# emmyoh/zebra

Hardware: AMD Instinct MI355X
Metric: queries/sec (higher is better)
Workload: dtype f32

## Files before the change

zebra_amd/csrc/zh_approx.hip:

```cpp

#include <cstdlib>

#include "zh_internal.h"
#include "zh_device.h"

typedef _Float16 f16x8 __attribute__((ext_vector_type(8)));

#ifndef ZH_APX_G768
#define ZH_APX_G768 2
#endif
#ifndef ZH_APX_G128
#define ZH_APX_G128 8
#endif
uint32_t zh_approx_groups(uint32_t d) {
    switch (d) {
    case 128: return ZH_APX_G128;
    case 256: case 384: return 4;
    case 768: return ZH_APX_G768;
    case 512: case 1024: return 2;
    default: return 0;
    }
}
bool zh_approx_pays(uint32_t d) { return d >= 384; }

float zh_approx_bound(int metric, uint32_t d, int mfma) {
    const double u = 5.9604644775390625e-8, c0 = (d + 255) / 256 + 8.0, ops = mfma ? 33.0 * (d / 128) + 2.0 + (mfma == 2 ? 40.0 : 0.0) : 0.0;
    if (metric == ZH_COSINE) return (float)(1.01 * (2.0 * c0 + 80.0 + 2.0 * ops) * u);
    return (float)(1.01 * (c0 + 100.0 + ops) * u);
}

__device__ __forceinline__ _Float16 f16_no_subnormal(float v) {
    const _Float16 h = (_Float16)v;
    return fabsf((float)h) < 6.103515625e-05f ? (_Float16)0.f : h;
}

template <int G>
__global__ __launch_bounds__(64) void qhalf_kernel(const float *__restrict__ Q, uint32_t B, uint32_t d, _Float16 *__restrict__ Qh,
                                                    float4 *__restrict__ qmeta) {
    constexpr uint32_t LG = 64 / G;
    const uint32_t b = blockIdx.x, lane = threadIdx.x;
    const float *q = Q + (size_t)b * d;
    float m = 0.f, s2 = 0.f;
    bool bad = false;
    for (uint32_t e = lane; e < d; e += 64) {
        const float v = q[e];
        bad |= !(v - v == 0.f);
        m = fmaxf(m, fabsf(v));
        s2 = __builtin_fmaf(v, v, s2);
    }
    m = wave_butterfly<OpMax>(m);
    s2 = wave_sum_canonical(s2);
    bad = __ballot(bad) != 0;
    float sigma = 1.f, inv = 1.f;
    if (!bad && m > 0.f) {
        int ex = 0;
        (void)frexpf(m, &ex);
        if (ex < -90 || ex > 90) bad = true;
        else { sigma = ldexpf(1.f, 14 - ex); inv = ldexpf(1.f, ex - 14); }
    }
    float d2 = 0.f;
    for (uint32_t e = lane; e < d; e += 64) {
        const float v = bad ? 0.f : q[e];
        const _Float16 h = f16_no_subnormal(v * sigma);
        const float df = v - (float)h * inv;
        d2 = __builtin_fmaf(df, df, d2);
        const uint32_t j = e / (4 * LG), rem = e % (4 * LG), l = rem / 4, t = rem % 4, i = j / 2, wh = j % 2;
        Qh[(size_t)b * d + ((size_t)(i * LG + l)) * 8 + wh * 4 + t] = h;
    }
    d2 = wave_sum_canonical(d2);
    if (lane == 0) {
        float4 o;
        if (bad || !(s2 - s2 == 0.f)) o = make_float4(NAN, NAN, NAN, NAN);
        else o = make_float4(inv, s2, sqrtf(s2) * (1.0f + 1e-5f), sqrtf(d2) * 1.001f);
        qmeta[b] = o;
    }
}

hipError_t zh_launch_qhalf(const float *dQ, uint32_t B, uint32_t d, void *dQh, float4 *dQmeta, int layout, hipStream_t s) {
    if (!B) return hipSuccess;
    const uint32_t G = layout == 2 ? 64 : (layout == 1 ? 16 : zh_approx_groups(d));
    if (G == 64) hipLaunchKernelGGL(qhalf_kernel<64>, dim3(B), dim3(64), 0, s, dQ, B, d, (_Float16 *)dQh, dQmeta);
    else if (G == 16) hipLaunchKernelGGL(qhalf_kernel<16>, dim3(B), dim3(64), 0, s, dQ, B, d, (_Float16 *)dQh, dQmeta);
    else if (G == 8) hipLaunchKernelGGL(qhalf_kernel<8>, dim3(B), dim3(64), 0, s, dQ, B, d, (_Float16 *)dQh, dQmeta);
    else if (G == 4) hipLaunchKernelGGL(qhalf_kernel<4>, dim3(B), dim3(64), 0, s, dQ, B, d, (_Float16 *)dQh, dQmeta);
    else if (G == 2) hipLaunchKernelGGL(qhalf_kernel<2>, dim3(B), dim3(64), 0, s, dQ, B, d, (_Float16 *)dQh, dQmeta);
    else return hipErrorInvalidValue;
    return hipGetLastError();
}

template <int LG>
__device__ __forceinline__ float group_sum(float s) {
    s = s + dpp_mov<0xB1>(s);
    s = s + dpp_mov<0x4E>(s);
    s = s + dpp_mov<0x141>(s);
    if (LG >= 16) s = s + dpp_mov<0x140>(s);
    if (LG >= 32) s = xor16<OpAdd>(s);
    if (LG >= 64) {
        const auto r = __builtin_amdgcn_permlane32_swap(__float_as_uint(s), __float_as_uint(s), false, false);
        s = __uint_as_float(r[0]) + __uint_as_float(r[1]);
    }
    return s;
}


__device__ __forceinline__ uint32_t scan_phase1(uint32_t lane, uint32_t n_ent, const uint2 *__restrict__ ent,
                                                const uint32_t *__restrict__ visitBits, const uint4 *__restrict__ nodeVisit,
                                                uint32_t *eGb, uint32_t *eWithin, uint32_t *eC, uint32_t *off, uint32_t *eB0, uint64_t *eK0) {
    unsigned long long rlw[ZH_SCAN_NE];
#pragma unroll
    for (int j = 0; j < ZH_SCAN_NE; j++) {
        const uint32_t e = lane + 64u * j;
        rlw[j] = __builtin_nontemporal_load(reinterpret_cast<const unsigned long long *>(ent + (e < n_ent ? e : 0)));
    }
    uint32_t word[ZH_SCAN_NE];
    bool in[ZH_SCAN_NE];
#pragma unroll
    for (int j = 0; j < ZH_SCAN_NE; j++) {
        const uint32_t node = (uint32_t)rlw[j];
        in[j] = lane + 64u * j < n_ent && node != 0xFFFFFFFFu;
        word[j] = visitBits[in[j] ? node >> 5 : 0];
    }
    uint4 nv[ZH_SCAN_NE];
#pragma unroll
    for (int j = 0; j < ZH_SCAN_NE; j++) {
        const uint32_t node = (uint32_t)rlw[j];
        in[j] = in[j] && ((word[j] >> (node & 31)) & 1u);
        nv[j] = nodeVisit[in[j] ? node : 0];
    }
    uint32_t P = 0;
#pragma unroll
    for (int j = 0; j < ZH_SCAN_NE; j++) {
        eWithin[j] = (uint32_t)(rlw[j] >> 32);
        eC[j] = in[j] ? nv[j].x & 0x0FFFFFFFu : 0u;
        eGb[j] = nv[j].y; eB0[j] = nv[j].z;
        eK0[j] = ((uint64_t)(nv[j].x >> 28) << 32) | nv[j].w;
        uint32_t incl = eC[j];
#pragma unroll
        for (int o = 1; o < 64; o <<= 1) {
            const uint32_t t = __shfl_up(incl, o);
            if (lane >= (uint32_t)o) incl += t;
        }
        off[j] = P + incl - eC[j];
        P += (uint32_t)__builtin_amdgcn_readlane((int)incl, 63);
    }
    return P;
}

#define ZH_APX_CAP 512
#ifndef ZH_APX_WAVES
#define ZH_APX_WAVES 0
#endif
#ifndef ZH_APX_REPL_ROWS
#define ZH_APX_REPL_ROWS 0
#endif
template <int D, int G, int KINDA>
__global__ __launch_bounds__(256)
#if ZH_APX_WAVES
__attribute__((amdgpu_waves_per_eu(ZH_APX_WAVES, 8)))
#endif
void scan_approx_kernel(const float *__restrict__ X, const uint4 *__restrict__ Qh,
                                                           const float4 *__restrict__ qmeta, const uint2 *__restrict__ rowLeaf,
                                                           uint32_t T, uint32_t RW, const uint32_t *__restrict__ visitBits,
                                                           const uint4 *__restrict__ nodeVisit, const ZhGroup *__restrict__ groups,
                                                           uint32_t GRP, uint64_t row_begin, uint64_t row_end, float Kc,
                                                           uint64_t *__restrict__ iv) {
    constexpr int LG = 64 / G, NH = D * G / 512, NR = 2 * NH;
    constexpr int RB = NR <= 6 ? 4 : 2;
    static_assert(D * G % 512 == 0 && NH >= 1, "a lane's share of a query is whole 16-byte loads");
    __shared__ uint4 pair_list[4][ZH_APX_CAP];
    __shared__ uint32_t row_start[4][20];
    const uint32_t lane = threadIdx.x & 63, l = lane & (LG - 1), g = lane / LG;
    const uint32_t wid = (uint32_t)__builtin_amdgcn_readfirstlane((int)(threadIdx.x >> 6));
    const uint64_t wave = (uint64_t)blockIdx.x * (blockDim.x >> 6) + wid;
    const uint64_t r0 = row_begin + wave * RW;
    if (r0 >= row_end) return;
    const uint32_t nr = (uint32_t)(row_end - r0 < RW ? row_end - r0 : RW);
    const uint32_t n_ent = nr * T;
    const uint2 *__restrict__ ent = rowLeaf + (size_t)r0 * T;
    uint32_t eGb[ZH_SCAN_NE], eWithin[ZH_SCAN_NE], eC[ZH_SCAN_NE], off[ZH_SCAN_NE], eB0[ZH_SCAN_NE];
    uint64_t eK0[ZH_SCAN_NE];
    const uint32_t P = scan_phase1(lane, n_ent, ent, visitBits, nodeVisit, eGb, eWithin, eC, off, eB0, eK0);
    if (P == 0) return;
    const float4 *__restrict__ X4 = reinterpret_cast<const float4 *>(X);
    float my_s = 0.f, my_a2 = 0.f;
    uint64_t my_slot = 0;
    uint32_t nst = 0;
    bool my_on = false;
    auto flush = [&]() {
        if (my_on) __builtin_nontemporal_store(((uint64_t)__float_as_uint(my_a2) << 32) | __float_as_uint(my_s), iv + my_slot);
        my_on = false;
        nst = 0;
    };
    auto load_q = [&](uint32_t b, uint4 *hq) {
        const uint4 *qp = Qh + (size_t)b * (D / 8) + l;
#pragma unroll
        for (int i = 0; i < NH; i++) hq[i] = qp[i * LG];
    };
    auto load_x = [&](uint64_t row, float4 *v) {
        if constexpr (G == 2 && !ZH_APX_REPL_ROWS) {
            const float4 *r4 = X4 + (size_t)row * (D / 4) + lane;
#pragma unroll
            for (int j = 0; j < NR / 2; j++) {
                const float4 t = ld16<true>(r4 + 64 * j);
                const auto sx = __builtin_amdgcn_permlane32_swap(__float_as_uint(t.x), __float_as_uint(t.x), false, false);
                const auto sy = __builtin_amdgcn_permlane32_swap(__float_as_uint(t.y), __float_as_uint(t.y), false, false);
                const auto sz = __builtin_amdgcn_permlane32_swap(__float_as_uint(t.z), __float_as_uint(t.z), false, false);
                const auto sw = __builtin_amdgcn_permlane32_swap(__float_as_uint(t.w), __float_as_uint(t.w), false, false);
                v[2 * j] = make_float4(__uint_as_float(sx[0]), __uint_as_float(sy[0]), __uint_as_float(sz[0]), __uint_as_float(sw[0]));
                v[2 * j + 1] = make_float4(__uint_as_float(sx[1]), __uint_as_float(sy[1]), __uint_as_float(sz[1]), __uint_as_float(sw[1]));
            }
        } else {
            const float4 *r4 = X4 + (size_t)row * (D / 4) + l;
#pragma unroll
            for (int j = 0; j < NR; j++) v[j] = ld16<true>(r4 + LG * j);
        }
    };
    auto row_sumsq = [&](const float4 *v) {
        float4 c = make_float4(0.f, 0.f, 0.f, 0.f);
#pragma unroll
        for (int j = 0; j < NR; j++) sq4(v[j], c);
        return group_sum<LG>((c.x + c.y) + (c.z + c.w));
    };
    auto dot_h = [&](const float4 *v, const uint4 *hq) {
        float ax = 0.f, ay = 0.f, az = 0.f, aw = 0.f;
#pragma unroll
        for (int i = 0; i < NH; i++) {
            f16x8 h;
            __builtin_memcpy(&h, &hq[i], 16);
            ax = __builtin_fmaf(v[2 * i].x, (float)h[0], ax);
            ay = __builtin_fmaf(v[2 * i].y, (float)h[1], ay);
            az = __builtin_fmaf(v[2 * i].z, (float)h[2], az);
            aw = __builtin_fmaf(v[2 * i].w, (float)h[3], aw);
            ax = __builtin_fmaf(v[2 * i + 1].x, (float)h[4], ax);
            ay = __builtin_fmaf(v[2 * i + 1].y, (float)h[5], ay);
            az = __builtin_fmaf(v[2 * i + 1].z, (float)h[6], az);
            aw = __builtin_fmaf(v[2 * i + 1].w, (float)h[7], aw);
        }
        return group_sum<LG>((ax + ay) + (az + aw));
    };
    auto stash = [&](float s, float a2, uint32_t, uint64_t slot, bool valid) {
        if (l == nst) { my_s = s; my_a2 = a2; my_slot = slot; my_on = valid; }
        if (++nst == (uint32_t)LG) flush();
    };
    if (P <= ZH_APX_CAP) {
        uint4 *list = pair_list[wid];
        uint32_t *rstart = row_start[wid];
        uint32_t mrows = 0;
#pragma unroll
        for (int j = 0; j < ZH_SCAN_NE; j++) {
            const uint32_t e = lane + 64u * j, c = eC[j];
            if (e < n_ent && e % T == 0) rstart[e / T] = off[j];
            if (c) {
                const uint32_t rl = e / T, gb = eGb[j];
                mrows |= 1u << rl;
                {
                    const uint64_t slot = eK0[j] + eWithin[j];
                    list[off[j]] = make_uint4(rl, eB0[j], (uint32_t)slot, (uint32_t)(slot >> 32));
                }
                for (uint32_t sidx = 1; sidx < c; sidx++) {
                    const ZhGroup *gp = groups + gb + sidx / GRP;
                    const uint64_t slot = gp->key_off[sidx % GRP] + eWithin[j];
                    list[off[j] + sidx] = make_uint4(rl, gp->b[sidx % GRP], (uint32_t)slot, (uint32_t)(slot >> 32));
                }
            }
        }
        if (lane == 0) rstart[nr] = P;
        uint32_t rowmask = 0;
#pragma unroll
        for (int bit = 0; bit < 16; bit++) rowmask |= (__ballot((mrows >> bit) & 1u) != 0 ? 1u : 0u) << bit;
        __builtin_amdgcn_fence(__ATOMIC_RELEASE, "wavefront");
        __builtin_amdgcn_wave_barrier();
        uint32_t p = 0;
        uint4 rec = list[g < P ? g : P - 1];
        uint4 hq[NH];
        load_q(rec.y, hq);
        while (rowmask) {
            uint32_t rid[RB];
#pragma unroll
            for (int r = 0; r < RB; r++) {
                rid[r] = rowmask ? (uint32_t)__builtin_ctz(rowmask) : 0xFFFFFFFFu;
                rowmask &= rowmask - 1;
            }
            float4 v[RB][NR];
#pragma unroll
            for (int r = 0; r < RB; r++)
                if (rid[r] != 0xFFFFFFFFu) load_x(r0 + rid[r], v[r]);
#pragma unroll
            for (int r = 0; r < RB; r++) {
                if (rid[r] == 0xFFFFFFFFu) continue;
                const uint32_t pb = (uint32_t)__builtin_amdgcn_readfirstlane((int)rstart[rid[r] + 1]);
                const float a2 = row_sumsq(v[r]);
                uint4 recn, hqn[NH];
                auto one = [&](const uint4 &ru, const uint4 *hu, uint4 &rp, uint4 *hp) {
                    const uint32_t pn = p + G < pb ? p + G : pb;
                    rp = list[pn + g < P ? pn + g : P - 1];
                    load_q(rp.y, hp);
                    const float s = dot_h(v[r], hu);
                    stash(s, a2, ru.y, ((uint64_t)ru.w << 32) | ru.z, p + g < pb);
                    p = pn;
                };
                while (p < pb) {
                    one(rec, hq, recn, hqn);
                    if (p < pb) one(recn, hqn, rec, hq);
                    else {
                        rec = recn;
#pragma unroll
                        for (int i = 0; i < NH; i++) hq[i] = hqn[i];
                    }
                }
            }
        }
    } else {
        float4 v[NR];
        float a2 = 0.f;
        uint32_t cur = 0xFFFFFFFFu;
#pragma unroll
        for (int j = 0; j < ZH_SCAN_NE; j++) {
            unsigned long long m = __ballot(eC[j] != 0);
            while (m) {
                const int ll = __builtin_ctzll(m);
                m &= m - 1;
                const uint32_t c = (uint32_t)__builtin_amdgcn_readlane((int)eC[j], ll);
                const uint32_t gb = (uint32_t)__builtin_amdgcn_readlane((int)eGb[j], ll);
                const uint32_t w = (uint32_t)__builtin_amdgcn_readlane((int)eWithin[j], ll);
                const uint32_t rl = ((uint32_t)ll + 64u * j) / T;
                if (rl != cur) {
                    cur = rl;
                    load_x(r0 + rl, v);
                    a2 = row_sumsq(v);
                }
                for (uint32_t s0 = 0; s0 < c; s0 += G) {
                    const uint32_t sidx = s0 + g < c ? s0 + g : c - 1;
                    const ZhGroup *gp = groups + gb + sidx / GRP;
                    const uint32_t b = gp->b[sidx % GRP];
                    uint4 hq[NH];
                    load_q(b, hq);
                    const float s = dot_h(v, hq);
                    stash(s, a2, b, gp->key_off[sidx % GRP] + w, s0 + g < c);
                }
            }
        }
    }
    flush();
}

typedef float f32x4v __attribute__((ext_vector_type(4)));
typedef uint32_t u32x4v __attribute__((ext_vector_type(4)));

__global__ __launch_bounds__(256) void row_half_kernel(const float *__restrict__ X, uint64_t row0, uint64_t n_rows, uint32_t d,
                                                       _Float16 *__restrict__ Xh, float2 *__restrict__ rowMeta, uint32_t *__restrict__ rhoMax,
                                                       const uint32_t *__restrict__ perm, uint64_t perm_rows) {
    const uint32_t lane = threadIdx.x & 63, NS = d / 32;
    const uint64_t nw = (uint64_t)gridDim.x * 4;
    float rho_w = 0.f;
    for (uint64_t i = (uint64_t)blockIdx.x * 4 + (threadIdx.x >> 6); i < n_rows; i += nw) {
        const uint64_t row = row0 + i;
        const float *x = X + (size_t)(perm && row < perm_rows ? perm[row] : row) * d;
        float m = 0.f, a2 = 0.f;
        bool bad = false;
        for (uint32_t e = lane; e < d; e += 64) {
            const float v = x[e];
            bad |= !(v - v == 0.f);
            m = fmaxf(m, fabsf(v));
            a2 = __builtin_fmaf(v, v, a2);
        }
        m = wave_butterfly<OpMax>(m);
        a2 = wave_sum_canonical(a2);
        bad = __ballot(bad) != 0;
        bool usable = false;
        float sigma = 1.f, inv = __uint_as_float(0x7FC00000u);
        if (!bad) {
            int ex = 14;
            if (m > 0.f) (void)frexpf(m, &ex);
            if (ex >= -100 && ex <= 100) { usable = true; sigma = ldexpf(1.f, 14 - ex); inv = ldexpf(1.f, ex - 14); }
        }
        float s2 = 0.f, d2 = 0.f;
        _Float16 *tile = Xh + ((size_t)(row >> 4) * NS * 64 + (row & 15)) * 8;
        for (uint32_t e = lane; e < d; e += 64) {
            const float v = x[e] * sigma;
            const _Float16 hv = usable ? f16_no_subnormal(v) : (_Float16)0.f;
            const float df = v - (float)hv;
            s2 = __builtin_fmaf(v, v, s2);
            d2 = __builtin_fmaf(df, df, d2);
            const uint32_t st = e >> 5, w = e & 31, hh = (w & 15) >> 2, j = (w & 3) + ((w >> 4) << 2);
            if (Xh) tile[((size_t)st * 64 + hh * 16) * 8 + j] = hv;
        }
        s2 = wave_sum_canonical(s2);
        d2 = wave_sum_canonical(d2);
        if (usable && s2 > 0.f) rho_w = fmaxf(rho_w, sqrtf(d2) * 1.001f / (sqrtf(s2) * 0.9999f));
        if (lane == 0) rowMeta[row] = make_float2(a2, inv);
    }
    if (lane == 0 && rho_w > 0.f) atomicMax(rhoMax, __float_as_uint(rho_w));
}

hipError_t zh_launch_row_half(const float *dX, uint64_t row0, uint64_t n_rows, uint32_t d, void *dXh, float2 *dRowMeta, uint32_t *dRhoMax,
                              const uint32_t *dPerm, uint64_t perm_rows, hipStream_t s) {
    if (!n_rows) return hipSuccess;
    const uint64_t blocks = std::min<uint64_t>((n_rows + 3) / 4, 256 * 32);
    hipLaunchKernelGGL(row_half_kernel, dim3((uint32_t)blocks), dim3(256), 0, s, dX, row0, n_rows, d, (_Float16 *)dXh, dRowMeta, dRhoMax, dPerm, perm_rows);
    return hipGetLastError();
}

__global__ __launch_bounds__(256) void permute_row_leaf_kernel(const uint2 *__restrict__ rowLeaf, const uint32_t *__restrict__ perm, uint64_t perm_rows,
                                                               uint64_t n_entries, uint32_t T, uint2 *__restrict__ out) {
    for (uint64_t e = (uint64_t)blockIdx.x * blockDim.x + threadIdx.x; e < n_entries; e += (uint64_t)gridDim.x * blockDim.x) {
        const uint64_t p = e / T, t = e % T;
        out[e] = rowLeaf[(size_t)(p < perm_rows ? perm[p] : p) * T + t];
    }
}
hipError_t zh_launch_permute_row_leaf(const uint2 *dRowLeaf, const uint32_t *dPerm, uint64_t perm_rows, uint64_t n_rows, uint32_t T, uint2 *dOut, hipStream_t s) {
    const uint64_t n = n_rows * T;
    if (!n) return hipSuccess;
    hipLaunchKernelGGL(permute_row_leaf_kernel, dim3((uint32_t)std::min<uint64_t>((n + 255) / 256, 256 * 64)), dim3(256), 0, s, dRowLeaf, dPerm, perm_rows, n, T, dOut);
    return hipGetLastError();
}

#ifndef ZH_MFMA_CL
#define ZH_MFMA_CL 0
#endif
#ifdef ZH_SCAN_GUARD
#define ZH_GUARD(cond, bit) ((cond) ? true : (atomicOr(guard, (bit)), false))
#else
#define ZH_GUARD(cond, bit) true
#endif
#ifdef ZH_SCAN_PROF
__device__ unsigned long long zh_scan_prof_buf[16];
extern "C" __attribute__((visibility("default"))) int zh_debug_scan_prof(uint64_t *out, uint32_t words, int reset) {
    static const unsigned long long zero[16] = {};
    if (reset) return (int)hipMemcpyToSymbol(HIP_SYMBOL(zh_scan_prof_buf), zero, sizeof(zero));
    return (int)hipMemcpyFromSymbol(out, HIP_SYMBOL(zh_scan_prof_buf), (size_t)words * 8);
}
#define SP(...) __VA_ARGS__
#else
#define SP(...)
#endif
#ifndef ZH_MFMA_WAVES
#define ZH_MFMA_WAVES 3
#endif
template <int D, bool F32ROWS>
__global__ __launch_bounds__(256) __attribute__((amdgpu_waves_per_eu(D > 768 ? 2 : ZH_MFMA_WAVES, D > 768 ? 2 : ZH_MFMA_WAVES)))
void scan_mfma_kernel(const u32x4v *__restrict__ Xh, const float *__restrict__ Xf, const float2 *__restrict__ rowMeta,
                                                         const uint4 *__restrict__ Qh, const uint2 *__restrict__ rowLeaf, uint32_t T,
                                                         uint32_t RW, const uint32_t *__restrict__ visitBits,
                                                         const uint4 *__restrict__ nodeVisit, const ZhGroup *__restrict__ groups,
                                                         uint32_t GRP, uint64_t row_begin, uint64_t row_end, uint64_t *__restrict__ iv,
                                                         uint32_t *__restrict__ colStats ,
                                                         uint32_t nq, uint64_t iv_cap, uint32_t *__restrict__ guard) {
    constexpr int NS = D / 32;
    constexpr int NL = D / 64;
    constexpr int CL = ZH_MFMA_CL ? ZH_MFMA_CL : (NL % 4 == 0 ? 2 : 3);
    constexpr int NCH = NL / CL;
    static_assert(D % 128 == 0 && NL % CL == 0 && NCH % 2 == 0, "four accumulators; the chunk registers alternate with a static parity");
    __shared__ uint64_t pair_list[4][ZH_APX_CAP > CL * 256 ? ZH_APX_CAP : CL * 256];
    __shared__ uint64_t tile_list[4][ZH_APX_CAP];
    __shared__ uint32_t col_query[4][ZH_APX_CAP];
    __shared__ uint32_t tile_start[4][36];
    __shared__ f32x4v acc_lds[4][64];
    __shared__ float2 row_meta[4][16];
    const uint32_t lane = threadIdx.x & 63, c16 = lane & 15, h = lane >> 4;
    const uint32_t wid = (uint32_t)__builtin_amdgcn_readfirstlane((int)(threadIdx.x >> 6));
    const uint64_t wave = (uint64_t)blockIdx.x * (blockDim.x >> 6) + wid;
    const uint64_t r0 = row_begin + wave * RW;
    if (r0 >= row_end) return;
    SP(const uint64_t sp0 = clock64();)
    const uint32_t nr = (uint32_t)(row_end - r0 < RW ? row_end - r0 : RW);
    const uint32_t n_ent = nr * T;
    const uint2 *__restrict__ ent = rowLeaf + (size_t)r0 * T;
    uint32_t eGb[ZH_SCAN_NE], eWithin[ZH_SCAN_NE], eC[ZH_SCAN_NE], off[ZH_SCAN_NE], eB0[ZH_SCAN_NE];
    uint64_t eK0[ZH_SCAN_NE];
    const uint32_t P = scan_phase1(lane, n_ent, ent, visitBits, nodeVisit, eGb, eWithin, eC, off, eB0, eK0);
    if (P == 0) return;
    SP(const uint64_t sp1 = clock64();)
    uint64_t *list = pair_list[wid];
    const bool listed = P <= ZH_APX_CAP;
    auto pack = [](uint32_t rl, uint32_t b, uint64_t slot) { return slot | ((uint64_t)b << 36) | ((uint64_t)rl << 60); };
#pragma unroll
    for (int j = 0; j < ZH_SCAN_NE; j++) {
        const uint32_t e = lane + 64u * j, c = eC[j];
        if (c && listed && ZH_GUARD(off[j] + c <= (uint32_t)ZH_APX_CAP && e / T < 16u, 32u)) {
            const uint32_t rl = e / T, gb = eGb[j];
            list[off[j]] = pack(rl, eB0[j], eK0[j] + eWithin[j]);
            for (uint32_t sidx = 1; sidx < c; sidx++) {
                const ZhGroup *gp = groups + gb + sidx / GRP;
                list[off[j] + sidx] = pack(rl, gp->b[sidx % GRP], gp->key_off[sidx % GRP] + eWithin[j]);
            }
        }
    }
    SP(__builtin_amdgcn_s_waitcnt(0); const uint64_t sp2 = clock64();)
    f16x8 A[NS];
    if constexpr (!F32ROWS) {
        const u32x4v *tp = Xh + (size_t)(r0 >> 4) * (NS * 64) + lane;
#pragma unroll
        for (int st = 0; st < NS; st++) A[st] = __builtin_bit_cast(f16x8, __builtin_nontemporal_load(tp + 64 * st));
        if (lane < 16) row_meta[wid][lane] = rowMeta[r0 + (lane < nr ? lane : 0u)];
        __builtin_amdgcn_fence(__ATOMIC_RELEASE, "wavefront");
        __builtin_amdgcn_wave_barrier();
    } else {
        if (lane < 16) row_meta[wid][lane] = rowMeta[r0 + (lane < nr ? lane : 0u)];
        __builtin_amdgcn_fence(__ATOMIC_RELEASE, "wavefront");
        __builtin_amdgcn_wave_barrier();
        const float inv_c = row_meta[wid][c16].y;
        const bool usable_c = inv_c - inv_c == 0.f;
        const float sigma_c = usable_c ? 1.0f / inv_c : 0.f;
        f32x4v *xt = reinterpret_cast<f32x4v *>(tile_list[wid]);
        const f32x4v *X4 = reinterpret_cast<const f32x4v *>(Xf);
        const uint32_t g4 = lane >> 4, p16 = lane & 15;
        auto cvt8 = [&](const f32x4v lo, const f32x4v hi) {
            f16x8 o;
#pragma unroll
            for (int t = 0; t < 4; t++) {
                o[t] = usable_c ? f16_no_subnormal(lo[t] * sigma_c) : (_Float16)0.f;
                o[4 + t] = usable_c ? f16_no_subnormal(hi[t] * sigma_c) : (_Float16)0.f;
            }
            return o;
        };
        f32x4v Rr[4];
        auto issue_rows = [&](int kb) {
#pragma unroll
            for (int i = 0; i < 4; i++) {
                const uint32_t rr = 4u * i + g4;
                Rr[i] = __builtin_nontemporal_load(X4 + (size_t)(r0 + (rr < nr ? rr : nr - 1)) * (D / 4) + kb * 16 + p16);
            }
        };
        issue_rows(0);
#pragma unroll
        for (int kb = 0; kb < D / 64; kb++) {
#pragma unroll
            for (int i = 0; i < 4; i++) {
                const uint32_t rr = 4u * i + g4;
                xt[rr * 16 + (p16 ^ rr)] = Rr[i];
            }
            __builtin_amdgcn_fence(__ATOMIC_RELEASE, "wavefront");
            __builtin_amdgcn_wave_barrier();
            if (kb + 1 < D / 64) issue_rows(kb + 1);
#pragma unroll
            for (int s2 = 0; s2 < 2; s2++) {
                const f32x4v lo = xt[c16 * 16 + ((8u * s2 + h) ^ c16)], hi = xt[c16 * 16 + ((8u * s2 + 4u + h) ^ c16)];
                A[2 * kb + s2] = cvt8(lo, hi);
            }
            __builtin_amdgcn_fence(__ATOMIC_RELEASE, "wavefront");
            __builtin_amdgcn_wave_barrier();
        }
    }
    const float2 *rmeta = row_meta[wid];
    u32x4v *stg = reinterpret_cast<u32x4v *>(pair_list[wid]);
    const u32x4v *__restrict__ Qv = reinterpret_cast<const u32x4v *>(Qh);
    const uint32_t g8 = lane >> 3, pc = lane & 7;
    const uint32_t swA = (g8 >> 1) & 7u, swB = (4u + (g8 >> 1)) & 7u;
    const uint32_t rd0 = (c16 >> 3) * 64u + (c16 & 7u) * 8u + ((h ^ (c16 >> 1)) & 7u);
    const uint32_t rd1 = (c16 >> 3) * 64u + (c16 & 7u) * 8u + (((4u + h) ^ (c16 >> 1)) & 7u);
    auto issue = [&](uint32_t bA, uint32_t bB, int chunk, u32x4v *dst) {
        if (!ZH_GUARD(bA < nq && bB < nq, 1u)) { bA = 0; bB = 0; }
        const u32x4v *qa = Qv + (size_t)bA * (D / 8) + (size_t)(chunk * CL * 8) + (pc ^ swA);
        const u32x4v *qb = Qv + (size_t)bB * (D / 8) + (size_t)(chunk * CL * 8) + (pc ^ swB);
#pragma unroll
        for (int i = 0; i < CL; i++) { dst[2 * i] = qa[8 * i]; dst[2 * i + 1] = qb[8 * i]; }
    };
    auto to_lds = [&](const u32x4v *src) {
#pragma unroll
        for (int i = 0; i < 2 * CL; i++) stg[64 * i + lane] = src[i];
    };
    auto mfma_chunk = [&](int chunk, f32x4v *acc) {
#pragma unroll
        for (int i = 0; i < 2 * CL; i++) {
            const u32x4v v = stg[128 * (i / 2) + ((i & 1) ? rd1 : rd0)];
            const int st = chunk * 2 * CL + i;
            acc[st & 3] = __builtin_amdgcn_mfma_f32_16x16x32_f16(A[st], __builtin_bit_cast(f16x8, v), acc[st & 3], 0, 0, 0);
        }
    };
    auto emit = [&](const f32x4v *acc, uint32_t rl, uint64_t slot, bool valid) {
        const f32x4v t = (acc[0] + acc[1]) + (acc[2] + acc[3]);
        if (valid && (rl >> 2) == h) {
            const uint32_t i = rl & 3u;
            const float sv = i == 0 ? t[0] : (i == 1 ? t[1] : (i == 2 ? t[2] : t[3]));
            const float2 rm = rmeta[rl];
            if (ZH_GUARD(slot < iv_cap, 2u))
                __builtin_nontemporal_store(((uint64_t)__float_as_uint(rm.x) << 32) | __float_as_uint(sv * rm.y), iv + slot);
        }
    };
    if (listed) {
        uint32_t *tab = reinterpret_cast<uint32_t *>(tile_list[wid]);
        uint32_t *colq = col_query[wid], *tstart = tile_start[wid];
#pragma unroll
        for (int i = 0; i < 4; i++) reinterpret_cast<uint4 *>(tab)[lane + 64 * i] = make_uint4(0u, 0u, 0u, 0u);
        if (lane < 36) tstart[lane] = 0u;
        __builtin_amdgcn_fence(__ATOMIC_RELEASE, "wavefront");
        __builtin_amdgcn_wave_barrier();
        auto hash_of = [](uint32_t b) { return (b * 2654435761u) >> 22; };
        uint32_t nd = 0;
        for (uint32_t p0 = 0; p0 < P; p0 += 64) {
            const uint32_t pi = p0 + lane;
            const bool valid = pi < P;
            const uint32_t b = valid ? (uint32_t)(list[pi] >> 36) & 0xFFFFFFu : 0u, key = b + 1u;
            uint32_t hs = hash_of(b);
            bool leader = false, open = valid;
            while (__ballot(open)) {
                if (open) {
                    const uint32_t old = atomicCAS(&tab[hs], 0u, (key << 9) | 0x1FFu);
                    if (old == 0u) { leader = true; open = false; }
                    else if ((old >> 9) == key) open = false;
                    else hs = (hs + 1u) & 1023u;
                }
            }
            const unsigned long long lm = __ballot(leader);
            if (leader) {
                const uint32_t col = nd + (uint32_t)__builtin_popcountll(lm & ((1ull << lane) - 1ull));
                if (ZH_GUARD(col < (uint32_t)ZH_APX_CAP && hs < 1024u, 64u)) {
                    tab[hs] = (key << 9) | col;
                    colq[col] = b;
                }
            }
            nd += (uint32_t)__builtin_popcountll(lm);
        }
        __builtin_amdgcn_fence(__ATOMIC_RELEASE, "wavefront");
        __builtin_amdgcn_wave_barrier();
        for (uint32_t p0 = 0; p0 < P; p0 += 64) {
            const uint32_t pi = p0 + lane;
            if (pi < P) {
                const uint64_t rec = list[pi];
                const uint32_t b = (uint32_t)(rec >> 36) & 0xFFFFFFu, key = b + 1u;
                uint32_t hs = hash_of(b), w = tab[hs];
                for (uint32_t tries = 0; (w >> 9) != key && ZH_GUARD(tries < 1024u, 16u); tries++) { (void)tries; hs = (hs + 1u) & 1023u; w = tab[hs]; }
                const uint32_t col = w & 0x1FFu;
                if (!ZH_GUARD((w >> 9) == key && col < nd, 128u)) continue;
                const uint32_t pos = atomicAdd(&tstart[1 + (col >> 4)], 1u);
                list[pi] = (rec & ~(0xFFFFFFull << 36)) | ((uint64_t)(col | (pos << 9)) << 36);
            }
        }
        __builtin_amdgcn_fence(__ATOMIC_RELEASE, "wavefront");
        __builtin_amdgcn_wave_barrier();
        {
            uint32_t v = lane < 33 ? tstart[lane] : 0u;
#pragma unroll
            for (int o = 1; o < 64; o <<= 1) {
                const uint32_t u = __shfl_up(v, o);
                if (lane >= (uint32_t)o) v += u;
            }
            __builtin_amdgcn_wave_barrier();
            if (lane < 33) tstart[lane] = v;
        }
        __builtin_amdgcn_fence(__ATOMIC_RELEASE, "wavefront");
        __builtin_amdgcn_wave_barrier();
        uint64_t *tl = tile_list[wid];
        {
            uint64_t recs[ZH_APX_CAP / 64];
#pragma unroll
            for (int i = 0; i < ZH_APX_CAP / 64; i++) recs[i] = (uint32_t)(64 * i) + lane < P ? list[64 * i + lane] : ~0ull;
            __builtin_amdgcn_wave_barrier();
#pragma unroll
            for (int i = 0; i < ZH_APX_CAP / 64; i++)
                if ((uint32_t)(64 * i) + lane < P) {
                    const uint32_t cp = (uint32_t)(recs[i] >> 36) & 0xFFFFFFu, col = cp & 0x1FFu, pos = (cp >> 9) & 0x1FFu;
                    if (ZH_GUARD(tstart[col >> 4] + pos < (uint32_t)ZH_APX_CAP && col < nd, 4u | (col < nd ? 0u : 8u))) tl[tstart[col >> 4] + pos] = recs[i];
                }
        }
        __builtin_amdgcn_fence(__ATOMIC_RELEASE, "wavefront");
        __builtin_amdgcn_wave_barrier();
        const uint32_t nt = (nd + 15) / 16;
        SP(const uint64_t sp3 = clock64();)
        if (colStats && lane == 0 && (wave & 63u) == 0u) { atomicAdd(&colStats[0], nd); atomicAdd(&colStats[1], P); }
        auto col_b = [&](uint32_t t, uint32_t col) { const uint32_t ci = 16 * t + col; return colq[ci < nd ? ci : nd - 1]; };
        uint32_t bA = col_b(0, g8), bB = col_b(0, 8 + g8);
        u32x4v ra[2 * CL], rb[2 * CL];
        issue(bA, bB, 0, ra);
        SP(__builtin_amdgcn_s_waitcnt(0); const uint64_t sp4 = clock64();)
        f32x4v *al = acc_lds[wid];
        for (uint32_t t = 0; t < nt; t++) {
            f32x4v acc[4] = {{0.f, 0.f, 0.f, 0.f}, {0.f, 0.f, 0.f, 0.f}, {0.f, 0.f, 0.f, 0.f}, {0.f, 0.f, 0.f, 0.f}};
#pragma unroll
            for (int c = 0; c < NCH; c += 2) {
                issue(bA, bB, c + 1, rb);
                to_lds(ra);
                mfma_chunk(c, acc);
                if (c + 2 < NCH) issue(bA, bB, c + 2, ra);
                else {
                    bA = col_b(t + 1, g8); bB = col_b(t + 1, 8 + g8);
                    issue(bA, bB, 0, ra);
                }
                to_lds(rb);
                mfma_chunk(c + 1, acc);
            }
            al[c16 * 4 + h] = (acc[0] + acc[1]) + (acc[2] + acc[3]);
            __builtin_amdgcn_fence(__ATOMIC_RELEASE, "wavefront");
            __builtin_amdgcn_wave_barrier();
            const uint32_t pe = tstart[t + 1];
            for (uint32_t pi = tstart[t] + lane; pi < pe; pi += 64) {
                const uint64_t rec = tl[pi];
                const uint32_t rl = (uint32_t)(rec >> 60), col = (uint32_t)(rec >> 36) & 15u;
                const float sv = reinterpret_cast<const float *>(al)[col * 16 + rl];
                const float2 rm = rmeta[rl];
                if (ZH_GUARD((rec & 0xFFFFFFFFFull) < iv_cap, 2u))
                    __builtin_nontemporal_store(((uint64_t)__float_as_uint(rm.x) << 32) | __float_as_uint(sv * rm.y), iv + (rec & 0xFFFFFFFFFull));
            }
            __builtin_amdgcn_wave_barrier();
        }
        SP(if ((wave & 15u) == 0u && lane == 0) {
            __builtin_amdgcn_s_waitcnt(0);
            const uint64_t sp5 = clock64();
            atomicAdd(&zh_scan_prof_buf[0], 1ull); atomicAdd(&zh_scan_prof_buf[1], sp1 - sp0); atomicAdd(&zh_scan_prof_buf[2], sp2 - sp1);
            atomicAdd(&zh_scan_prof_buf[3], sp3 - sp2); atomicAdd(&zh_scan_prof_buf[4], sp4 - sp3); atomicAdd(&zh_scan_prof_buf[5], sp5 - sp4);
            atomicAdd(&zh_scan_prof_buf[6], (unsigned long long)nt); atomicAdd(&zh_scan_prof_buf[7], (unsigned long long)P);
            atomicAdd(&zh_scan_prof_buf[8], (unsigned long long)nd); atomicAdd(&zh_scan_prof_buf[9], sp5 - sp0);
        })
    } else {
#pragma unroll
        for (int j = 0; j < ZH_SCAN_NE; j++) {
            unsigned long long m = __ballot(eC[j] != 0);
            while (m) {
                const int ll = __builtin_ctzll(m);
                m &= m - 1;
                const uint32_t c = (uint32_t)__builtin_amdgcn_readlane((int)eC[j], ll);
                const uint32_t gb = (uint32_t)__builtin_amdgcn_readlane((int)eGb[j], ll);
                const uint32_t w = (uint32_t)__builtin_amdgcn_readlane((int)eWithin[j], ll);
                const uint32_t rl = ((uint32_t)ll + 64u * j) / T;
                for (uint32_t s0 = 0; s0 < c; s0 += 16) {
                    auto visit_b = [&](uint32_t col) { const uint32_t si = s0 + col < c ? s0 + col : c - 1; return groups[gb + si / GRP].b[si % GRP]; };
                    const uint32_t bA = visit_b(g8), bB = visit_b(8 + g8);
                    const uint32_t sidx = s0 + c16 < c ? s0 + c16 : c - 1;
                    const ZhGroup *gp = groups + gb + sidx / GRP;
                    f32x4v acc[4] = {{0.f, 0.f, 0.f, 0.f}, {0.f, 0.f, 0.f, 0.f}, {0.f, 0.f, 0.f, 0.f}, {0.f, 0.f, 0.f, 0.f}};
                    u32x4v rq[2 * CL];
#pragma unroll
                    for (int cc = 0; cc < NCH; cc++) {
                        issue(bA, bB, cc, rq);
                        to_lds(rq);
                        mfma_chunk(cc, acc);
                        __builtin_amdgcn_sched_barrier(0);
                    }
                    emit(acc, rl, gp->key_off[sidx % GRP] + w, s0 + c16 < c);
                }
            }
        }
    }
}

template <int D>
static hipError_t launch_scan_mfma_d(const float *dX, uint64_t n_rows, const ZhApprox &ap, const uint2 *dRowLeaf, uint32_t T,
                                     const uint32_t *dVisitBits, const uint4 *dNodeVisit, const ZhGroup *dGroups, uint32_t group, hipStream_t s) {
    const uint32_t RW = zh_scan_rows_per_wave(T);
    uint64_t rows_per_launch = zh_sweep_rows_per_launch(D);
    rows_per_launch = rows_per_launch / (4 * RW) * (4 * RW);
    for (uint64_t r = 0; r < n_rows; r += rows_per_launch) {
        const uint64_t r_end = r + rows_per_launch < n_rows ? r + rows_per_launch : n_rows;
        const uint64_t waves = (r_end - r + RW - 1) / RW, blocks = (waves + 3) / 4;
        if (blocks > 0x7FFFFFFFull) return hipErrorInvalidValue;
        if (ap.row_half)
            hipLaunchKernelGGL((scan_mfma_kernel<D, false>), dim3((uint32_t)blocks), dim3(256), 0, s, (const u32x4v *)ap.row_half, dX, ap.row_meta, (const uint4 *)ap.Qh, dRowLeaf, T, RW,
                               dVisitBits, dNodeVisit, dGroups, group, r, r_end, ap.iv, ap.ctl + 5, ap.n_queries, ap.iv_cap, ap.ctl + 7);
        else
            hipLaunchKernelGGL((scan_mfma_kernel<D, true>), dim3((uint32_t)blocks), dim3(256), 0, s, (const u32x4v *)nullptr, dX, ap.row_meta, (const uint4 *)ap.Qh, dRowLeaf, T, RW,
                               dVisitBits, dNodeVisit, dGroups, group, r, r_end, ap.iv, ap.ctl + 5, ap.n_queries, ap.iv_cap, ap.ctl + 7);
    }
    return hipGetLastError();
}

__global__ __launch_bounds__(256) void absmax_kernel(const float *__restrict__ X, uint64_t n, uint32_t *__restrict__ out) {
    float m = 0.f;
    for (uint64_t i = (uint64_t)blockIdx.x * blockDim.x + threadIdx.x; i < n; i += (uint64_t)gridDim.x * blockDim.x) {
        const float v = fabsf(X[i]);
        if (v - v == 0.f) m = fmaxf(m, v);
    }
    m = wave_butterfly<OpMax>(m);
    if ((threadIdx.x & 63) == 0 && m > 0.f) atomicMax(out, __float_as_uint(m));
}

__global__ __launch_bounds__(256) void row_half128_kernel(const float *__restrict__ X, uint64_t row0, uint64_t n_rows, float sigma,
                                                          _Float16 *__restrict__ Xh, uint32_t *__restrict__ rhoMax) {
    const uint32_t lane = threadIdx.x & 63;
    const uint64_t nw = (uint64_t)gridDim.x * 4;
    float rho_w = 0.f;
    for (uint64_t i = (uint64_t)blockIdx.x * 4 + (threadIdx.x >> 6); i < n_rows; i += nw) {
        const uint64_t row = row0 + i;
        const float2 x = reinterpret_cast<const float2 *>(X + (size_t)row * 128)[lane];
        const float v0 = x.x * sigma, v1 = x.y * sigma;
        bool bad = !(v0 - v0 == 0.f) || !(v1 - v1 == 0.f) || fabsf(v0) > 60000.f || fabsf(v1) > 60000.f;
        const _Float16 h0 = f16_no_subnormal(v0), h1 = f16_no_subnormal(v1);
        const float d0 = v0 - (float)h0, d1 = v1 - (float)h1;
        const float s2 = wave_sum_canonical(__builtin_fmaf(v0, v0, v1 * v1));
        const float d2 = wave_sum_canonical(__builtin_fmaf(d0, d0, d1 * d1));
        const float m = wave_butterfly<OpMax>(fmaxf(fabsf(x.x), fabsf(x.y)));
        bad = __ballot(bad) != 0 || !(s2 - s2 == 0.f) || (s2 == 0.f && m > 0.f);
        const float rho = s2 > 0.f ? sqrtf(d2) * 1.001f / (sqrtf(s2) * 0.9999f) : 0.f;
        bad = bad || !(rho <= 9.765625e-4f);
        if (!bad) rho_w = fmaxf(rho_w, rho);
        const _Float16 nanh = (_Float16)__uint_as_float(0x7FC00000u);
        typedef _Float16 f16x2v __attribute__((ext_vector_type(2)));
        reinterpret_cast<f16x2v *>(Xh + (size_t)row * 128)[lane] = bad ? f16x2v{nanh, nanh} : f16x2v{h0, h1};
    }
    if (lane == 0 && rho_w > 0.f) atomicMax(rhoMax, __float_as_uint(rho_w));
}

hipError_t zh_launch_absmax(const float *dX, uint64_t n, uint32_t *dOut, hipStream_t s) {
    if (!n) return hipSuccess;
    hipLaunchKernelGGL(absmax_kernel, dim3((uint32_t)std::min<uint64_t>((n + 255) / 256, 256 * 16)), dim3(256), 0, s, dX, n, dOut);
    return hipGetLastError();
}
hipError_t zh_launch_row_half128(const float *dX, uint64_t row0, uint64_t n_rows, float sigma, void *dXh, uint32_t *dRhoMax, hipStream_t s) {
// ... 1631 lines not shown
```

Baseline: 204,600.

## Prefetch row tiles during scan phase and parallelize pair-list expansion across lanes

The fp16 row tile and row metadata loads are issued right after the entry loads inside scan_phase1, so their latency overlaps the visit-bit and node lookups. An opaque-pointer trick and a scheduling barrier keep the compiler from sinking these loads. Pair-list expansion no longer has each lane loop serially over its entry's slots. Each lane now writes a descriptor and a start mark in LDS, and a wave-wide prefix-max scan lets every list slot find its owning entry and fill itself in parallel, in two unrolled rounds. This adds LDS traffic, shuffles and register pressure from holding A[] live through phase one.

```diff
diff --git a/zebra_amd/csrc/zh_approx.hip b/zebra_amd/csrc/zh_approx.hip
--- a/zebra_amd/csrc/zh_approx.hip
+++ b/zebra_amd/csrc/zh_approx.hip
@@ -103,15 +103,19 @@
 }
 
 
+struct ZhNothing { __device__ __forceinline__ void operator()() const {} };
+template <class Behind = ZhNothing>
 __device__ __forceinline__ uint32_t scan_phase1(uint32_t lane, uint32_t n_ent, const uint2 *__restrict__ ent,
                                                 const uint32_t *__restrict__ visitBits, const uint4 *__restrict__ nodeVisit,
-                                                uint32_t *eGb, uint32_t *eWithin, uint32_t *eC, uint32_t *off, uint32_t *eB0, uint64_t *eK0) {
+                                                uint32_t *eGb, uint32_t *eWithin, uint32_t *eC, uint32_t *off, uint32_t *eB0, uint64_t *eK0,
+                                                Behind behind_entries = Behind()) {
     unsigned long long rlw[ZH_SCAN_NE];
 #pragma unroll
     for (int j = 0; j < ZH_SCAN_NE; j++) {
         const uint32_t e = lane + 64u * j;
         rlw[j] = __builtin_nontemporal_load(reinterpret_cast<const unsigned long long *>(ent + (e < n_ent ? e : 0)));
     }
+    behind_entries();
     uint32_t word[ZH_SCAN_NE];
     bool in[ZH_SCAN_NE];
 #pragma unroll
@@ -437,6 +441,12 @@
 #ifndef ZH_MFMA_WAVES
 #define ZH_MFMA_WAVES 3
 #endif
+template <class V>
+__device__ __forceinline__ const __attribute__((address_space(1))) V *zh_opaque_global(const V *p) {
+    uint64_t a = (uint64_t)p;
+    asm volatile("" : "+v"(a));
+    return (const __attribute__((address_space(1))) V *)a;
+}
 template <int D, bool F32ROWS>
 __global__ __launch_bounds__(256) __attribute__((amdgpu_waves_per_eu(D > 768 ? 2 : ZH_MFMA_WAVES, D > 768 ? 2 : ZH_MFMA_WAVES)))
 void scan_mfma_kernel(const u32x4v *__restrict__ Xh, const float *__restrict__ Xf, const float2 *__restrict__ rowMeta,
@@ -468,31 +478,86 @@
     const uint2 *__restrict__ ent = rowLeaf + (size_t)r0 * T;
     uint32_t eGb[ZH_SCAN_NE], eWithin[ZH_SCAN_NE], eC[ZH_SCAN_NE], off[ZH_SCAN_NE], eB0[ZH_SCAN_NE];
     uint64_t eK0[ZH_SCAN_NE];
-    const uint32_t P = scan_phase1(lane, n_ent, ent, visitBits, nodeVisit, eGb, eWithin, eC, off, eB0, eK0);
+    f16x8 A[NS];
+    float2 rm_lane;
+    const uint32_t P = scan_phase1(lane, n_ent, ent, visitBits, nodeVisit, eGb, eWithin, eC, off, eB0, eK0, [&]() {
+        if constexpr (!F32ROWS) {
+            const auto *tp = zh_opaque_global(Xh + (size_t)(r0 >> 4) * (NS * 64) + lane);
+#pragma unroll
+            for (int st = 0; st < NS; st++) A[st] = __builtin_bit_cast(f16x8, __builtin_nontemporal_load(tp + 64 * st));
+            const unsigned long long rmw = *zh_opaque_global(reinterpret_cast<const unsigned long long *>(rowMeta + r0 + (lane < nr ? lane : 0u)));
+            rm_lane = make_float2(__uint_as_float((uint32_t)rmw), __uint_as_float((uint32_t)(rmw >> 32)));
+            asm volatile("" ::: "memory");
+            __builtin_amdgcn_sched_barrier(0);
+        }
+    });
     if (P == 0) return;
     SP(const uint64_t sp1 = clock64();)
     uint64_t *list = pair_list[wid];
     const bool listed = P <= ZH_APX_CAP;
     auto pack = [](uint32_t rl, uint32_t b, uint64_t slot) { return slot | ((uint64_t)b << 36) | ((uint64_t)rl << 60); };
-#pragma unroll
-    for (int j = 0; j < ZH_SCAN_NE; j++) {
-        const uint32_t e = lane + 64u * j, c = eC[j];
-        if (c && listed && ZH_GUARD(off[j] + c <= (uint32_t)ZH_APX_CAP && e / T < 16u, 32u)) {
-            const uint32_t rl = e / T, gb = eGb[j];
-            list[off[j]] = pack(rl, eB0[j], eK0[j] + eWithin[j]);
-            for (uint32_t sidx = 1; sidx < c; sidx++) {
-                const ZhGroup *gp = groups + gb + sidx / GRP;
-                list[off[j] + sidx] = pack(rl, gp->b[sidx % GRP], gp->key_off[sidx % GRP] + eWithin[j]);
-            }
-        }
+    if (listed) {
+        static_assert(64 * ZH_SCAN_NE * sizeof(uint4) <= sizeof(tile_list[0]), "a descriptor per entry of the wave");
+        uint4 *desc = reinterpret_cast<uint4 *>(tile_list[wid]);
+        uint32_t *mark = col_query[wid];
+#pragma unroll
+        for (int i = 0; i < ZH_APX_CAP / 64; i++)
+            if (64u * i < P) mark[64 * i + lane] = 0u;
+        __builtin_amdgcn_fence(__ATOMIC_RELEASE, "wavefront");
+        __builtin_amdgcn_wave_barrier();
+#pragma unroll
+        for (int j = 0; j < ZH_SCAN_NE; j++) {
+            const uint32_t e = lane + 64u * j, c = eC[j];
+            if (c && ZH_GUARD(off[j] + c <= (uint32_t)ZH_APX_CAP && e / T < 16u, 32u)) {
+                const uint32_t rl = e / T;
+                list[off[j]] = pack(rl, eB0[j], eK0[j] + eWithin[j]);
+                desc[e] = make_uint4(off[j], c | (rl << 28), eGb[j], eWithin[j]);
+                mark[off[j]] = e + 1u;
+            }
+        }
+        __builtin_amdgcn_fence(__ATOMIC_RELEASE, "wavefront");
+        __builtin_amdgcn_wave_barrier();
+        uint32_t carry = 0;
+        auto rounds = [&](uint32_t pb) {
+            uint32_t rlv[4], qb[4], ew[4];
+            uint64_t ko[4];
+#pragma unroll
+            for (int i = 0; i < 4; i++) {
+                const uint32_t p = pb + 64u * i + lane;
+                uint32_t m = p < P ? mark[p] : 0u;
+#pragma unroll
+                for (int o = 1; o < 64; o <<= 1) {
+                    const uint32_t t = __shfl_up(m, o);
+                    if (lane >= (uint32_t)o) m = m > t ? m : t;
+                }
+                m = m > carry ? m : carry;
+                carry = (uint32_t)__builtin_amdgcn_readlane((int)m, 63);
+                rlv[i] = 0u;
+                if (p < P && ZH_GUARD(m != 0u, 32u)) {
+                    const uint4 dsc = desc[m - 1u];
+                    const uint32_t sidx = p - dsc.x;
+                    if (sidx >= 1u && ZH_GUARD(sidx < (dsc.y & 0x0FFFFFFFu), 32u)) {
+                        const ZhGroup *gp = groups + dsc.z + sidx / GRP;
+                        qb[i] = gp->b[sidx % GRP];
+                        ko[i] = gp->key_off[sidx % GRP];
+                        ew[i] = dsc.w;
+                        rlv[i] = 0x80000000u | (dsc.y >> 28);
+                    }
+                }
+            }
+#pragma unroll
+            for (int i = 0; i < 4; i++) {
+                const uint32_t p = pb + 64u * i + lane;
+                if (rlv[i] && ZH_GUARD(p < (uint32_t)ZH_APX_CAP, 4u)) list[p] = pack(rlv[i] & 15u, qb[i], ko[i] + ew[i]);
+            }
+        };
+        static_assert(ZH_APX_CAP == 512, "two calls (not a loop: around a back edge every round would wait for the loads of the round before)");
+        rounds(0u);
+        if (P > 256u) rounds(256u);
     }
     SP(__builtin_amdgcn_s_waitcnt(0); const uint64_t sp2 = clock64();)
-    f16x8 A[NS];
     if constexpr (!F32ROWS) {
-        const u32x4v *tp = Xh + (size_t)(r0 >> 4) * (NS * 64) + lane;
-#pragma unroll
-        for (int st = 0; st < NS; st++) A[st] = __builtin_bit_cast(f16x8, __builtin_nontemporal_load(tp + 64 * st));
-        if (lane < 16) row_meta[wid][lane] = rowMeta[r0 + (lane < nr ? lane : 0u)];
+        if (lane < 16) row_meta[wid][lane] = rm_lane;
         __builtin_amdgcn_fence(__ATOMIC_RELEASE, "wavefront");
         __builtin_amdgcn_wave_barrier();
     } else {
```

Result: slower. 201,200 (-1.7%).
